# DhayaaAnbajagane/Baryonification

Hardware: AMD Instinct MI355X
Metric: halos/sec for BaryonifyShell NSIDE=1024 (1000000-halo synthetic catalog) (higher is better)
Workload: dtype f64 throughout in the parity-grade mode: f64 ring-row geometry, f64 pair math with 1e-11 elementary functions (fp32 seeds + one Newton step), f64 LDS accumulation, pix_offsets stored as two f32 arrays (hi + lo), f64 regrid geometry, f64 map

## Files before the change

baryonification_amd/csrc/bfgx_api.hip:

```cpp
#include <hip/hip_runtime.h>
#include <cmath>
#include <cstdarg>
#include <cstdio>
#include <algorithm>
#include <atomic>
#include <climits>
#include <cstdint>
#include <cstdlib>
#include <chrono>
#include <cstring>
#include <functional>
#include <map>
#include <memory>
#include <mutex>
#include <string>
#include <tuple>
#include <type_traits>
#include <vector>

#include "../../include/bfgx.h"

#include "bfgx_devmem.hpp"
#include "bfgx_tile_arena.hpp"
#include "bfgx_cosmo.hpp"
// ... 770 lines not shown
    {
        int cus = 0;
        if (hipDeviceGetAttribute(&cus, hipDeviceAttributeMultiprocessorCount, device) == hipSuccess && cus > 0) p->num_cus = cus;
    }
    p->nside = nside;
    p->max_halos = max_halos;
    p->hpx = make_hpx(nside);
    p->stream = (hipStream_t)hip_stream;
    auto bail = [&](int rc) { bfgx_plan_destroy(p); return rc; };

    const bfgx_table &t = model->table;
    if (int rc = upload_model(p->mem, p->stream, model, true, p->model, p->NC)) return bail(rc);
    plan_pick_precision(p, model);
    const size_t nh = (size_t)(max_halos > 0 ? max_halos : 1);
    if (p->mem.alloc(p->recs, nh)) return bail(alloc_fail("halo records"));
    if (p->NC > 4 && p->mem.alloc(p->rowsx, nh)) return bail(alloc_fail("corner rows"));
    if (int rc = plan_init_fast(p, t, nh)) return bail(rc);
    if (int rc = plan_init_binning(p, t, nh)) return bail(rc);
    if (int rc = plan_init_regrid(p)) return bail(rc);
    const ScanScratchLayout SL = scan_scratch_layout();
    int32_t *scan = nullptr;
    if (p->mem.alloc(scan, SL.total_words)) return bail(alloc_fail("tile scan scratch"));
    p->scan.bind(scan, SL);
    if (p->mem.alloc(p->tile_sums, 2 * (size_t)(p->tiling.ntiles + 1) + kFarEvalWgs)) return bail(alloc_fail("tile sums"));
    p->far_src.sums = p->tile_sums + 2 * (size_t)(p->tiling.ntiles + 1);
    if (hipMemsetAsync(p->far_src.sums, 0, sizeof(double) * kFarEvalWgs, p->stream) != hipSuccess) return bail(fail(BFGX_ERR_HIP, "hipMemset failed"));
    if (hipMemsetAsync(p->overflow, 0, sizeof(int32_t), p->stream) != hipSuccess) return bail(fail(BFGX_ERR_HIP, "hipMemset failed"));
    if (hipStreamSynchronize(p->stream) != hipSuccess) return bail(fail(BFGX_ERR_HIP, "stream sync failed"));
    *out = p;
    return BFGX_OK;
}

int bfgx_plan_timing_enable(bfgx_plan *p, int on)
{
    return p ? p->events.enable(on) : fail(BFGX_ERR_INVALID, "NULL plan");
}

int bfgx_plan_timing_read(bfgx_plan *p, double *ms_sum, int64_t *launches)
{
    return p ? p->events.read(p->device, p->stream, ms_sum, launches) : fail(BFGX_ERR_INVALID, "NULL argument");
}

void bfgx_plan_destroy(bfgx_plan *p)
{
    if (!p) return;
    (void)hipSetDevice(p->device);
    (void)hipStreamSynchronize(p->stream);
    p->events.destroy();
    p->mem.release();
// ... 171 lines not shown

}

constexpr int kSumTilesOneWg = 16384;
static int launch_tile_sums(bfgx_plan *p, int t0, int nt, double *sums_dev)
{
    const double *ts = p->tile_sums + 2 * (size_t)t0;
    const double *fs = p->far_src.sums;
    if (nt <= kSumTilesOneWg) hipLaunchKernelGGL(sum_tiles_kernel, dim3(1), dim3(256), 0, p->stream, nt, ts, sums_dev, fs, kFarEvalWgs);
    else {
        HIP_TRY(hipMemsetAsync(sums_dev, 0, 2 * sizeof(double), p->stream));
        hipLaunchKernelGGL(sum_tiles_multi_kernel, dim3(64), dim3(256), 0, p->stream, nt, ts, sums_dev, fs, kFarEvalWgs);
    }
    return BFGX_OK;
}

template <typename ACC, typename real, bool SPLIT = false>
static void launch_regrid_gather(bfgx_plan *p, const double *map_in_dev, const ACC *o, const ACC *o_lo, double *map_out_dev, double *ts, bool from_k1, double *sums_dev)
{
    const size_t lds = regrid3_lds_bytes(p->tiling.BR, p->tiling.W, sizeof(real)),
                 lds_walk = regrid3_lds_bytes(p->tiling.BR, p->tiling.W, sizeof(real), true, SPLIT ? sizeof(ACC) : sizeof(real));
    FarList far = p->far;
    far.overflow = p->arena.far_overflow_full;
    const int nt = p->tiling.ntiles, nfix = std::min(nt, 2 * p->num_cus), nwalk = std::min(nt, 4 * p->num_cus);
    const ReachArgs reach = reach_args(p, regrid_cap(p->hpx.nside));
    if (!from_k1)
        hipLaunchKernelGGL(tile_reach_kernel<ACC>, dim3(nt), dim3(256), 0, p->stream, p->hpx, p->tiling, o, p->arena.omax);
    hipLaunchKernelGGL(tile_apron_kernel, dim3((nt + 255) / 256), dim3(256), 0, p->stream, p->hpx, p->tiling, (const float *)p->arena.omax, 0,
                       reach.cap, 0, nt, p->tile_apron, p->arena.todo, p->regrid_lean);
    hipLaunchKernelGGL((tile_regrid3_kernel<ACC, real, 0, SPLIT>), dim3(std::min(nt, 8 * p->num_cus)), dim3(256), lds, p->stream, p->hpx, p->tiling, map_in_dev, o, o_lo,
                       map_out_dev, far, p->far_src, reach, ts, -1, nt, p->regrid_lean, (double *)nullptr);
    hipLaunchKernelGGL((tile_regrid3_kernel<ACC, real, 2, SPLIT>), dim3(nwalk), dim3(256), lds_walk, p->stream, p->hpx, p->tiling, map_in_dev, o, o_lo,
                       map_out_dev, far, p->far_src, reach, ts, -1, nt, p->arena.todo, (double *)nullptr);
    hipLaunchKernelGGL((regrid_far_eval_kernel<ACC, SPLIT>), dim3(kFarEvalWgs), dim3(256), 0, p->stream, p->hpx, p->tiling.rings, map_in_dev, o, o_lo, p->far_src, far);
    const bool many = nt > kSumTilesOneWg && sums_dev != nullptr && ts != nullptr;
    hipLaunchKernelGGL((tile_regrid3_kernel<ACC, real, 1, SPLIT>), dim3(nfix), dim3(256), lds, p->stream, p->hpx, p->tiling, map_in_dev, o, o_lo,
                       map_out_dev, far, p->far_src, reach, ts, -1, nt, p->arena.todo, many ? (double *)nullptr : sums_dev, p->regrid_lean);
    if (many) (void)launch_tile_sums(p, 0, nt, sums_dev);
}

extern "C" {

static int regrid_impl(bfgx_plan *p, const double *map_in_dev, const void *offsets_dev, const DispMode &m, double *map_out_dev, double *sums_dev,
                       bool from_k1)
{
    HIP_TRY(hipSetDevice(p->device));
    {
    KernelTimer kt(p, BFGX_K_REGRID);
    if (p->algo == 1) {
        if (!from_k1) HIP_TRY(hipMemsetAsync(p->arena.ctrl, 0, sizeof(RegridCtrl), p->stream));
        double *ts = sums_dev ? p->tile_sums : nullptr;
        if (m.split())
            launch_regrid_gather<float, double, true>(p, map_in_dev, (const float *)offsets_dev, m.lo(offsets_dev, p->hpx.npix),
                                                      map_out_dev, ts, from_k1, sums_dev);
        else if (m.fp64()) launch_regrid_gather<double, double>(p, map_in_dev, (const double *)offsets_dev, (const double *)nullptr, map_out_dev, ts, from_k1, sums_dev);
        else launch_regrid_gather<float, float>(p, map_in_dev, (const float *)offsets_dev, (const float *)nullptr, map_out_dev, ts, from_k1, sums_dev);
    } else {
        const unsigned grid = (unsigned)((p->hpx.npix + 255) / 256);
        if (m.fp64())
            hipLaunchKernelGGL(regrid_kernel<double>, dim3(grid), dim3(256), 0, p->stream, p->hpx, map_in_dev,
// ... 529 lines not shown
```

baryonification_amd/csrc/bfgx_regrid2.hpp:

```cpp
#pragma once
#include "bfgx_kernels.hpp"
#include "bfgx_scatter2.hpp"

namespace bfgx {

template <typename real>
struct alignas(16) RegRowC {
    real z, sth, dphi, inv_dphi;
    real c0, s0;
    real inv_dth_up, inv_dth_dn;
};
template <>
struct alignas(16) RegRowC<double> { double inv_dth_up, inv_dth_dn; };
template <typename real> struct RowGeom { real z, sth, dphi, inv_dphi, c0, s0, inv_dth_up, inv_dth_dn; };
__device__ inline RowGeom<float> row_geom(const RegRow *, const RegRowC<float> *rowc, int t)
{
    const RegRowC<float> c = rowc[t];
    return RowGeom<float>{c.z, c.sth, c.dphi, c.inv_dphi, c.c0, c.s0, c.inv_dth_up, c.inv_dth_dn};
}
__device__ inline RowGeom<double> row_geom(const RegRow *rows, const RegRowC<double> *rowc, int t)
{
    const RegRow &r = rows[t];
    const RegRowC<double> c = rowc[t];
    return RowGeom<double>{r.z, r.sth, r.dphi, r.inv_dphi, r.c0, r.s0, c.inv_dth_up, c.inv_dth_dn};
// ... 11 lines not shown
    __device__ inline double theta(int ir) const { return rows[ir - rth0].theta; }
    __device__ inline GenRing ring(int ir) const
    {
        const int t2 = ir - rth0;
        if (t2 >= 0 && t2 < LR + 2) { const RegRow &r2 = rows[t2]; return GenRing{r2.theta, r2.inv_dphi, r2.nr, r2.shf != 0}; }
        const RingRec &g2 = rings[ir];
        return GenRing{g2.theta, g2.inv_dphi, g2.nr, g2.shifted != 0};
    }
    __device__ inline GenSrc source(int ti, int x) const
    {
        const RegRow &rw = rows[ti];
        return GenSrc{rw.theta, rw.z, rw.sth, rw.dphi, rth0 + ti, rw.ks + x, rw.shf != 0};
    }
};
constexpr int kGenWalk = 17;
struct GenTable {
    const RingRec *__restrict__ rings; int lo_, hi_;
    __device__ inline int lo() const { return lo_; }
    __device__ inline int hi() const { return hi_; }
    __device__ inline double theta(int ir) const { return rings[ir].theta; }
    __device__ inline GenRing ring(int ir) const { const RingRec &g2 = rings[ir]; return GenRing{g2.theta, g2.inv_dphi, g2.nr, g2.shifted != 0}; }
};

template <typename RS>
__device__ inline void regrid_targets_generic(const Hpx &h, const RS &rs, const GenSrc &src, double o0, double o1, double o2, int tr[4], int tk[4], double w[4])
{
    const int nl4 = (int)(4 * h.nside);
    const double z = src.z, sth = src.sth;
    const double phi = ((double)src.k + (src.shf ? 0.5 : 0.0)) * src.dphi;
    double s, c;
    sincos_bounded(phi, s, c);
    const double nx = sth * c + o0, ny = sth * s + o1, nz = z + o2;
    const double xr = nx * c + ny * s, yr = ny * c - nx * s;
    const double inv = fast_rsq(nx * nx + ny * ny + nz * nz);
    const double zc = nz * inv;
    const double tq = yr * fast_rcp(xr);
    const double sn = fast_sqrt(xr * xr + yr * yr) * inv;
    const double q = sn * z - zc * sth;
    double theta, ph;
    if (xr > 0.0 && fabs(tq) <= 0.1 && fabs(q) <= 0.05) {
        ph = phi + atan_small(tq);
        theta = src.theta + asin_small(q);
    } else {
        theta = atan2_generic(sn, zc);
        ph = atan2_generic(ny, nx);
    }
    if (ph < 0) ph += kTwoPi;
    if (ph >= kTwoPi) ph -= kTwoPi;
    const int rlo = rs.lo(), rhi = rs.hi();
    const int rz = (int)ring_above(h, zc);
    int r1 = rz < rlo ? rlo : (rz > rhi ? rhi : rz);
    while (r1 > rlo && theta < rs.theta(r1)) --r1;
    while (r1 < rhi && theta >= rs.theta(r1 + 1)) ++r1;
    const bool in_window = (theta >= rs.theta(r1)) && (r1 < rhi) && (theta < rs.theta(r1 + 1));
    const int ir1 = in_window ? r1 : rz;
    const int ir2 = ir1 + 1;
    double theta1 = 0.0, theta2 = 0.0;
    for (int q4 = 0; q4 < 4; ++q4) { tr[q4] = 0; tk[q4] = 0; w[q4] = 0.0; }
#pragma unroll
    for (int half = 0; half < 2; ++half) {
        const int ir = half ? ir2 : ir1;
        if (half ? (ir < nl4) : (ir > 0)) {
            const GenRing g2 = rs.ring(ir);
            const int n2 = g2.nr;
            const double shd = g2.shf ? 0.5 : 0.0, invd = g2.inv_dphi, th = g2.theta;
            const double tmp = ph * invd - shd;
            int j1 = (int)floor(tmp);
            const double w1 = tmp - (double)j1;
            int j2 = j1 + 1;
            if (j1 < 0) j1 += n2;
            if (j2 >= n2) j2 -= n2;
            tr[2 * half] = ir; tr[2 * half + 1] = ir;
            tk[2 * half] = j1; tk[2 * half + 1] = j2;
            w[2 * half] = 1.0 - w1; w[2 * half + 1] = w1;
            if (half) theta2 = th; else theta1 = th;
        }
    }
    if (ir1 == 0) {
        const double wtheta = theta / theta2;
        w[2] *= wtheta; w[3] *= wtheta;
        const double fac = (1.0 - wtheta) * 0.25;
        w[0] = fac; w[1] = fac; w[2] += fac; w[3] += fac;
        tr[0] = 1; tr[1] = 1; tk[0] = (tk[2] + 2) & 3; tk[1] = (tk[3] + 2) & 3;
    } else if (ir2 == nl4) {
        const double wtheta = (theta - theta1) / (kPi - theta1);
        w[0] *= (1.0 - wtheta); w[1] *= (1.0 - wtheta);
        const double fac = wtheta * 0.25;
        w[0] += fac; w[1] += fac; w[2] = fac; w[3] = fac;
        tr[2] = nl4 - 1; tr[3] = nl4 - 1; tk[2] = (tk[0] + 2) & 3; tk[3] = (tk[1] + 2) & 3;
    } else {
        const double wtheta = (theta - theta1) * fast_rcp(theta2 - theta1);
        w[0] *= (1.0 - wtheta); w[1] *= (1.0 - wtheta);
        w[2] *= wtheta; w[3] *= wtheta;
    }
}

__device__ inline float abs_(float v) { return __builtin_fabsf(v); }
__device__ inline double abs_(double v) { return __builtin_fabs(v); }
template <typename real> struct RMath;
template <> struct RMath<float> {
    static __device__ inline float rcp(float x) { const float y = __builtin_amdgcn_rcpf(x); return y * __builtin_fmaf(-x, y, 2.0f); }
    static __device__ inline float inv_norm(float e) { return fma_(e, fma_(e, fma_(e, fma_(e, 0.2734375f, -0.3125f), 0.375f), -0.5f), 1.0f); }
    static __device__ inline float sqrt1pm1(float t2) { return t2 * fma_(t2, fma_(t2, 0.0625f, -0.125f), 0.5f); }
    static __device__ inline float asin_(float q) { const float q2 = q * q; return q * fma_(q2, fma_(q2, fma_(q2, (float)(15.0 / 336.0), 0.075f), (float)(1.0 / 6.0)), 1.0f); }
    static __device__ inline float atan_(float t) { const float t2 = t * t; return t * fma_(t2, fma_(t2, fma_(t2, fma_(t2, (float)(1.0 / 9.0), (float)(-1.0 / 7.0)), 0.2f), (float)(-1.0 / 3.0)), 1.0f); }
};
template <> struct RMath<double> {
    static __device__ inline double rcp(double x) { return fast_rcp(x); }
    static __device__ inline double inv_norm(double e) { return fast_rsq(1.0 + e); }
    static __device__ inline double sqrt1pm1(double t2) { const double h = 1.0 + t2; return t2 * fast_rcp(1.0 + h * fast_rsq(h)); }
    static __device__ inline double asin_(double q) { return asin_small(q); }
    static __device__ inline double atan_(double t) { return atan_small(t); }
};

struct RMathE {
    static __device__ inline double rcp(double x) { const double y = (double)__builtin_amdgcn_rcpf((float)x); return __builtin_fma(y, __builtin_fma(-x, y, 1.0), y); }
    static __device__ inline double inv_norm(double e)
    {
        const double x = 1.0 + e, y = (double)__builtin_amdgcn_rsqf((float)x);
// ... 24 lines not shown
    return R > kReachMax ? kReachMax : R;
}
__host__ __device__ inline double regrid_cap_for_rings(int64_t nside, int R)
{
    const double c = 0.999 * (double)R / (1.5 * (double)nside), cap = regrid_cap(nside);
    return (R >= kReachMax || c > cap) ? cap : c;
}

struct alignas(16) RowScan {
    int32_t start, nr, ks, span;
    float need2, cf2, lim2;
    int32_t klr;
};

struct FarList {
    unsigned long long *count;
    int64_t *pix;
    double *val;
    int64_t cap;
    int32_t *overflow;
};

constexpr int kFarEvalWgs = 1024;
struct FarSrc {
    unsigned int *count;
    int2 *ent;
    int64_t cap;
    double *sums;
};

__device__ inline bool far_src_append(const FarSrc &fs, int ring, int k)
{
    const unsigned long long act = __ballot(1);
    const int rank = (int)__builtin_amdgcn_mbcnt_hi((unsigned)(act >> 32), __builtin_amdgcn_mbcnt_lo((unsigned)act, 0u));
    const int leader = __ffsll((long long)act) - 1;
    unsigned base = 0;
    if (rank == 0) base = atomicAdd(fs.count, (unsigned)__popcll(act));
    base = (unsigned)__shfl((int)base, leader, kWave);
    const unsigned i = base + (unsigned)rank;
    if ((int64_t)i >= fs.cap) return false;
    fs.ent[i] = make_int2(ring, k);
    return true;
}

struct ReachArgs {
    const int32_t *apron;
// ... 206 lines not shown
    const int tx = nr_ ? ti : t1, ty = nr_ ? (down ? ti + 1 : ti - 1) : t1 + 1;
    int jx, jy; real wx, wy;
    if (nr_) {
        const real wall = dph * rc.inv_dphi, f = __builtin_floor(wall);
        wx = wall - f; jx = kown + (int)f;
    } else {
        other_ring(tx, jx, wx);
    }
    other_ring(ty, jy, wy);
    const int nrx = rows[tx].nr, nry = rows[ty].nr;
    int jx2 = jx + 1, jy2 = jy + 1;
    jx = jx < 0 ? jx + nrx : (jx >= nrx ? jx - nrx : jx);
    jx2 = jx2 < 0 ? jx2 + nrx : (jx2 >= nrx ? jx2 - nrx : jx2);
    jy = jy < 0 ? jy + nry : (jy >= nry ? jy - nry : jy);
    jy2 = jy2 < 0 ? jy2 + nry : (jy2 >= nry ? jy2 - nry : jy2);
    const real wtx = x_upper ? (real)1 - wtheta : wtheta, wty = (real)1 - wtx;
    tt[0] = tx; tt[1] = tx; tk[0] = jx; tk[1] = jx2;
    w[0] = ((real)1 - wx) * wtx; w[1] = wx * wtx;
    tt[2] = ty; tt[3] = ty; tk[2] = jy; tk[3] = jy2;
    w[2] = ((real)1 - wy) * wty; w[3] = wy * wty;
    return true;
}

template <typename RS>
__device__ inline double regrid_far_pixel(const Hpx &h, const RingRec *__restrict__ rings, const RS &rs, const GenSrc &src, double o0, double o1, double o2,
                                          double val, FarList far)
{
    int tr[4], tk[4];
    double w[4], tot = 0.0;
    regrid_targets_generic(h, rs, src, o0, o1, o2, tr, tk, w);
    const unsigned long long act = __ballot(1);
    const int rank = (int)__builtin_amdgcn_mbcnt_hi((unsigned)(act >> 32), __builtin_amdgcn_mbcnt_lo((unsigned)act, 0u));
    const int leader = __ffsll((long long)act) - 1;
    unsigned long long base = 0;
    if (rank == 0) base = atomicAdd(far.count, 4ull * (unsigned long long)__popcll(act));
    base = ((unsigned long long)(unsigned)__shfl((int)(base >> 32), leader, kWave) << 32) | (unsigned)__shfl((int)base, leader, kWave);
    for (int q4 = 0; q4 < 4; ++q4) {
        const double v = w[q4] * val;
        const unsigned long long i = base + 4ull * (unsigned long long)rank + (unsigned long long)q4;
        if ((int64_t)i < far.cap) { far.pix[i] = rings[tr[q4]].start + tk[q4]; far.val[i] = v; } else atomicOr(far.overflow, 1);
        tot += v;
    }
    return tot;
}

constexpr int kK2Occ = 4;
template <typename ACC, typename real, int PASS, bool SPLIT = false>
__global__ void __launch_bounds__(256, kK2Occ)
tile_regrid3_kernel(Hpx h, Tiling T, const double *__restrict__ map_in, const ACC *__restrict__ offsets, const ACC *__restrict__ offsets_lo,
                    double *__restrict__ map_out, FarList far, FarSrc fsrc, ReachArgs reach, double *__restrict__ tile_sums, int tile_off, int ntiles,
                    int *__restrict__ todo, double *__restrict__ sums_out, int *__restrict__ lean_reset = nullptr)
{
    static_assert(!SPLIT || (sizeof(ACC) == 4 && sizeof(real) == 8), "split pix_offsets: fp32 halves, fp64 geometry");
    extern __shared__ __align__(16) unsigned char smem[];
    const int NTmax = T.BR + 2 * kReachMax + 2;
    double *acc = reinterpret_cast<double *>(smem);
    RegRow *rows = reinterpret_cast<RegRow *>(acc + T.BR * T.W);
    RegRowC<real> *rowc = reinterpret_cast<RegRowC<real> *>(rows + NTmax);
    const int tid = threadIdx.x;
    const int nl4 = (int)(4 * h.nside);
    if (PASS == 1 && lean_reset != nullptr && blockIdx.x == 0 && tid == 0) *lean_reset = 0;
    if (PASS == 1 && sums_out != nullptr && blockIdx.x == 0) {
        double sa = 0.0, sb = 0.0;
        for (int i = tid; i < ntiles; i += 256) { sa += tile_sums[2 * (int64_t)i]; sb += tile_sums[2 * (int64_t)i + 1]; }
        for (int i = tid; i < kFarEvalWgs; i += 256) sb += fsrc.sums[i];
#pragma unroll
        for (int sft = kWave >> 1; sft > 0; sft >>= 1) { sa += __shfl_down(sa, sft, kWave); sb += __shfl_down(sb, sft, kWave); }
        double *red = reinterpret_cast<double *>(smem);
        if ((tid & (kWave - 1)) == 0) { red[2 * (tid / kWave)] = sa; red[2 * (tid / kWave) + 1] = sb; }
        __syncthreads();
        if (tid == 0) {
            double ta = 0.0, tb = 0.0;
            for (int w = 0; w < 256 / kWave; ++w) { ta += red[2 * w]; tb += red[2 * w + 1]; }
            sums_out[0] = ta; sums_out[1] = tb;
        }
        __syncthreads();
    }
    if (PASS == 1 && *far.overflow == 0) {
        const unsigned long long n = *far.count;
        for (unsigned long long i = (unsigned long long)blockIdx.x * 256 + tid; i < n; i += (unsigned long long)gridDim.x * 256)
            atomicAdd(map_out + far.pix[i], far.val[i]);
        return;
    }
    const bool listed = (PASS == 2 || PASS == 0) && todo != nullptr;
    if (listed) ntiles = min(todo[0], ntiles);
    for (int blk = blockIdx.x; blk < ntiles; blk += ((PASS == 0 && !listed) ? ntiles : (int)gridDim.x)) {
    const int tile = listed ? todo[1 + blk] : ((tile_off < 0) ? T.tile_order[blk] : tile_off + blk);
    const int band = T.tile_band[tile];
    const int nphi = T.band_nphi[band];
    const int tj = tile - T.band_tile0[band];
    const int i0 = 1 + band * T.BR;
    const int i1 = min(i0 + T.BR, nl4);
    double sum_in = 0.0, sum_out = 0.0;
    __syncthreads();

    const int R = (PASS == 2) ? reach.apron[2 * tile] : 1;
    const int kap = (PASS == 1 || nphi == 1) ? 0 : reach.apron[2 * tile + 1];
    if (PASS == 0 && reach.apron[2 * tile] > 1) continue;
    if (PASS == 0 && reach.apron[2 * tile] == 0) {
        const int lane = tid & (kWave - 1), wid = tid / kWave;
        for (int rr = wid; rr < i1 - i0; rr += 256 / kWave) {
            const int64_t st = T.rings[i0 + rr].start;
            const int nr = T.rings[i0 + rr].nr, ks = tile_ks(tj, nr, nphi), ke = tile_ks(tj + 1, nr, nphi);
            for (int k = ks + lane; k < ke; k += kWave) {
                const double v = map_in[st + k];
                const double dep = (v > 0.0) ? v : 0.0;
// ... 290 lines not shown
        const int n = rt.ke - rt.ks;
        for (int xx = lane; xx < n; xx += kWave) {
            const double v = acc[rr * T.W + xx];
            dst[xx] = v;
            sum_out += v;
        }
    }
    if (tile_sums) {
        __syncthreads();
#pragma unroll
        for (int sft = kWave >> 1; sft > 0; sft >>= 1) { sum_in += __shfl_down(sum_in, sft, kWave); sum_out += __shfl_down(sum_out, sft, kWave); }
        if (lane == 0) { acc[2 * wid] = sum_in; acc[2 * wid + 1] = sum_out; }
        __syncthreads();
        if (tid == 0) {
            double sa_ = 0.0, sb_ = 0.0;
            for (int wv = 0; wv < 256 / kWave; ++wv) { sa_ += acc[2 * wv]; sb_ += acc[2 * wv + 1]; }
            tile_sums[2 * (int64_t)tile] = sa_; tile_sums[2 * (int64_t)tile + 1] = sb_;
        }
    }
    __syncthreads();
    }
}

template <typename ACC, bool SPLIT>
__global__ void __launch_bounds__(256)
regrid_far_eval_kernel(Hpx h, const RingRec *__restrict__ rings, const double *__restrict__ map_in, const ACC *__restrict__ offsets,
                       const ACC *__restrict__ offsets_lo, FarSrc fsrc, FarList far)
{
    __shared__ double red[256 / kWave];
    const int tid = threadIdx.x;
    const unsigned listed = *fsrc.count;
    if (listed == 0u) {
        if (tid == 0) fsrc.sums[blockIdx.x] = 0.0;
        return;
    }
    const unsigned n = (int64_t)listed < fsrc.cap ? listed : (unsigned)fsrc.cap;
    if (listed > n && blockIdx.x == 0 && tid == 0) atomicAdd(far.count, 4ull * (unsigned long long)(listed - n));
    const int nl4 = (int)(4 * h.nside);
    double tot = 0.0;
    for (unsigned i = blockIdx.x * 256u + (unsigned)tid; i < n; i += (unsigned)kFarEvalWgs * 256u) {
        const int2 e = fsrc.ent[i];
        const RingRec &g = rings[e.x];
        const int64_t p = g.start + e.y;
        double o0 = (double)offsets[3 * p + 0], o1 = (double)offsets[3 * p + 1], o2 = (double)offsets[3 * p + 2];
        if (SPLIT) { o0 += (double)offsets_lo[3 * p + 0]; o1 += (double)offsets_lo[3 * p + 1]; o2 += (double)offsets_lo[3 * p + 2]; }
        const GenTable rs{rings, max(e.x - kGenWalk, 0), min(e.x + kGenWalk, nl4)};
        const GenSrc src{g.theta, g.z, g.sth, g.dphi, e.x, e.y, g.shifted != 0};
        tot += regrid_far_pixel(h, rings, rs, src, o0, o1, o2, map_in[p], far);
    }
#pragma unroll
    for (int sft = kWave >> 1; sft > 0; sft >>= 1) tot += __shfl_down(tot, sft, kWave);
    if ((tid & (kWave - 1)) == 0) red[tid / kWave] = tot;
    __syncthreads();
    if (tid == 0) {
        double t = 0.0;
        for (int w = 0; w < 256 / kWave; ++w) t += red[w];
        fsrc.sums[blockIdx.x] = t;
    }
}

__global__ void __launch_bounds__(256)
regrid_far_local_kernel(FarList far, double *__restrict__ out_slice, int64_t p0, int64_t p1, unsigned long long *__restrict__ foreign,
                        int ntiles = 0, const double *__restrict__ tile_sums = nullptr, double *__restrict__ sums = nullptr,
                        const double *__restrict__ far_sums = nullptr)
{
    if (tile_sums != nullptr && blockIdx.x == gridDim.x - 1) {
        __shared__ double sa[256 / kWave], sb[256 / kWave];
        double xa = 0.0, xb = 0.0;
        for (int t = threadIdx.x; t < ntiles; t += 256) { xa += tile_sums[2 * t]; xb += tile_sums[2 * t + 1]; }
        if (far_sums != nullptr) for (int t = threadIdx.x; t < kFarEvalWgs; t += 256) xb += far_sums[t];
#pragma unroll
        for (int sft = kWave >> 1; sft > 0; sft >>= 1) { xa += __shfl_down(xa, sft, kWave); xb += __shfl_down(xb, sft, kWave); }
        const int lane = threadIdx.x & (kWave - 1), wid = threadIdx.x / kWave;
        if (lane == 0) { sa[wid] = xa; sb[wid] = xb; }
        __syncthreads();
        if (threadIdx.x == 0) {
            double ta = 0.0, tb = 0.0;
            for (int w = 0; w < 256 / kWave; ++w) { ta += sa[w]; tb += sb[w]; }
            sums[0] = ta; sums[1] = tb;
        }
// ... 12 lines not shown
```

baryonification_amd/csrc/bfgx_shell_bands.inc:

```

extern "C" {

int bfgx_plan_bands(bfgx_plan *p, int32_t *nbands, int64_t *band_first_pixel)
{
    if (!p || !nbands) return fail(BFGX_ERR_INVALID, "NULL argument");
    *nbands = p->tiling.nbands;
    if (band_first_pixel)
        for (int b = 0; b <= p->tiling.nbands; ++b) band_first_pixel[b] = band_range(p, b, b).p0;
    return BFGX_OK;
}

int bfgx_plan_band_apron(bfgx_plan *p, int32_t band0, int32_t band1, int64_t *olo, int64_t *ohi)
{
    if (!p || !olo || !ohi) return fail(BFGX_ERR_INVALID, "NULL argument");
    if (int rc = check_band_range(p, band0, band1)) return rc;
    const int64_t i0 = 1 + (int64_t)p->tiling.BR * band0, i1 = 1 + (int64_t)p->tiling.BR * band1;
    *olo = ring_first_pixel(p->hpx, i0 - p->band_reach);
    *ohi = ring_first_pixel(p->hpx, i1 + p->band_reach);
    return BFGX_OK;
}

int bfgx_plan_reach_rings(bfgx_plan *p, double max_offset, int32_t *rings)
{
    if (!p || !rings) return fail(BFGX_ERR_INVALID, "NULL argument");
// ... 26 lines not shown
    if (!map_in_dev || !offsets_dev || !out_slice_dev) return fail(BFGX_ERR_INVALID, "NULL argument");
    if (olo > need_lo || ohi < need_hi || olo < 0 || ohi > p->hpx.npix)
        return fail(BFGX_ERR_INVALID, "pix_offsets range [%lld, %lld) does not cover the bands and %d ring(s) either side [%lld, %lld)",
                    (long long)olo, (long long)ohi, p->band_reach, (long long)need_lo, (long long)need_hi);
    HIP_TRY(hipSetDevice(p->device));
    if (reset_far) HIP_TRY(hipMemsetAsync(p->far.count, 0, kFarCountersBytes, p->stream));
    else if (!src_zeroed) HIP_TRY(hipMemsetAsync(p->far_src.count, 0, sizeof(uint32_t), p->stream));
    const BandRange r = band_range(p, band0, band1);
    {
        KernelTimer kt(p, BFGX_K_REGRID);
        const size_t lds = regrid3_lds_bytes(p->tiling.BR, p->tiling.W, m.fp64() ? sizeof(double) : sizeof(float), p->band_reach > 1,
                                             m.split() ? sizeof(float) : 0);
        double *out_base = out_slice_dev - r.p0;
        const ReachArgs reach = reach_args(p, regrid_cap_for_rings(p->hpx.nside, p->band_reach));
        hipLaunchKernelGGL(tile_apron_kernel, dim3((r.nt + 255) / 256), dim3(256), 0, p->stream, p->hpx, p->tiling, (const float *)nullptr,
                           p->band_reach, reach.cap, r.t0, r.nt, p->tile_apron, (int32_t *)nullptr);
        double *ts = sums_dev ? p->tile_sums : nullptr;
        const dim3 grid(r.nt), blk(256);
        int *none = nullptr;
#define BFGX_REGRID3(ACC, REAL, SPLIT, OL)                                                                                                     \
        do {                                                                                                                                    \
            const ACC *o = (const ACC *)offsets_dev - 3 * olo;                                                                                  \
            if (p->band_reach == 1) hipLaunchKernelGGL((tile_regrid3_kernel<ACC, REAL, 0, SPLIT>), grid, blk, lds, p->stream, p->hpx, p->tiling, map_in_dev, o, OL, \
                                                       out_base, p->far, p->far_src, reach, ts, r.t0, r.nt, none, (double *)nullptr);           \
            else hipLaunchKernelGGL((tile_regrid3_kernel<ACC, REAL, 2, SPLIT>), grid, blk, lds, p->stream, p->hpx, p->tiling, map_in_dev, o, OL, \
                                    out_base, p->far, p->far_src, reach, ts, r.t0, r.nt, none, (double *)nullptr);                              \
            hipLaunchKernelGGL((regrid_far_eval_kernel<ACC, SPLIT>), dim3(kFarEvalWgs), blk, 0, p->stream, p->hpx, p->tiling.rings, map_in_dev, o, OL, p->far_src, p->far); \
        } while (0)
        if (m.split()) BFGX_REGRID3(float, double, true, m.lo(offsets_dev, ohi - olo) - 3 * olo);
        else if (m.fp64()) BFGX_REGRID3(double, double, false, (const double *)nullptr);
        else BFGX_REGRID3(float, float, false, (const float *)nullptr);
#undef BFGX_REGRID3
        HIP_TRY(hipGetLastError());
    }
    if (sums_dev && !sums_later) {
        KernelTimer kt(p, BFGX_K_SUM);
        if (int rc = launch_tile_sums(p, r.t0, r.nt, sums_dev)) return rc;
        HIP_TRY(hipGetLastError());
    }
    return BFGX_OK;
}

static int offsets_bands(bfgx_plan *p, const bfgx_catalog *cat, int32_t band0, int32_t band1, void *slice, const DispMode &m)
{
    const BandRange r = band_range(p, band0, band1);
    TileLaunch k1;
    k1.tile_lo = r.t0; k1.tile_n = r.nt;
    if (int rc = launch_k0(p, cat, 1, m.fp64())) return rc;
    k1.omax = p->arena.omax;
    return launch_offsets(p, m, slice, r.p0, r.p1, k1);
// ... 120 lines not shown
```

baryonification_amd/csrc/bfgx_tile_arena.hpp:

```cpp
#pragma once
#include <cstddef>
#include <cstdint>

namespace bfgx {

struct RegridCtrl {
    unsigned long long far_count;
    uint32_t far_src_count;
    int32_t spare[3];
    int32_t far_overflow_full;
    int32_t todo_count;
};
static_assert(sizeof(RegridCtrl) == 32 && alignof(RegridCtrl) == 8, "RegridCtrl is eight words, the first two a 64-bit counter");
static_assert(offsetof(RegridCtrl, far_src_count) == 8 && offsetof(RegridCtrl, todo_count) == 28, "the two list counters are adjacent; the todo count is the last word");

constexpr size_t kFarCountersBytes = offsetof(RegridCtrl, far_src_count) + sizeof(uint32_t);
constexpr size_t kCtrlWords =sizeof(RegridCtrl) / sizeof(int32_t);
constexpr size_t round_up4(size_t words) { return (words + 3) & ~(size_t)3; }

struct TileArenaLayout {
    size_t cnt_a_pad, cnt_b, cur_b, tile_counter, omax, ctrl, far_overflow_full, todo, todo_list, band_overflow;
    size_t cursor_words;
    size_t zeroed_words;
    size_t tail_words;
    size_t total_words;
};

constexpr TileArenaLayout tile_arena_layout(size_t ntiles, size_t cnt_pad)
{
    const size_t blk = ntiles + 1;
    TileArenaLayout L{};
    L.cnt_a_pad = 0;
// ... 46 lines not shown
{
    ScanScratchLayout L{};
    L.block_tot = 0;
    L.block_off = L.block_tot + kScanBlocksRoom;
    L.total_words = L.block_off + kScanBlocksRoom;
    return L;
}
struct ScanScratch {
    int32_t *block_tot = nullptr, *block_off = nullptr;
    void bind(int32_t *b, const ScanScratchLayout &L) { block_tot = b + L.block_tot; block_off = b + L.block_off; }
};

template <size_t NT, size_t PAD>
struct TileArenaCheck {
    static constexpr TileArenaLayout L = tile_arena_layout(NT, PAD);
    static constexpr size_t blk = NT + 1;
    static constexpr bool unrounded = (NT * PAD) % 4 == 0;
    static constexpr size_t n3p = round_up4(3 * blk + 1);
    static_assert(L.cnt_a_pad == 0 && L.cnt_b >= NT * PAD, "the padded counters start the arena and hold ntiles * cnt_pad words");
    static_assert(L.cur_b == L.cnt_b + blk && L.cursor_words == blk && L.tile_counter == L.cur_b + L.cursor_words,
                  "cnt_b and cur_b: ntiles + 1 words each, and nothing else lies in the cursors' span");
    static_assert(L.omax == L.tile_counter + 1, "the |offset|^2 block follows the tile counter");
    static_assert(L.ctrl >= L.omax + blk && L.ctrl - (L.omax + blk) < 4, "the control words follow the three blocks and the tile counter, rounded up to four words");
    static_assert(L.far_overflow_full == L.ctrl + 6 && L.todo == L.ctrl + 7 && L.todo_list == L.todo + 1, "count (64 bits), source count, three spare, overflow, todo count, todo tiles");
    static_assert(L.band_overflow == L.todo_list + NT && L.total_words > L.band_overflow, "the banded overflow flag follows the todo tiles, inside the allocation");
    static_assert(L.zeroed_words == L.ctrl + kCtrlWords, "the zeroed span starts at the base and ends exactly after RegridCtrl");
    static_assert(L.zeroed_words % 4 == 0, "the zeroed span is a multiple of 16 bytes");
    static_assert(L.todo_list >= L.zeroed_words && L.band_overflow >= L.zeroed_words, "the step's memset touches neither the todo tiles nor the banded overflow flag");
    static_assert(L.ctrl % 2 == 0, "RegridCtrl's 64-bit counter is 8-byte aligned (the base is a device allocation)");
    static_assert(L.tail_words == L.total_words - L.ctrl && L.tail_words == NT + 12, "plan creation zeroes the control words and all behind them");
    static_assert(L.cnt_b == round_up4(NT * PAD) && (!unrounded || L.cnt_b == NT * PAD), "only a padded region that is no multiple of four words is rounded up");
    static_assert(L.tile_counter == L.cnt_b + 2 * blk && L.omax == L.cnt_b + 2 * blk + 1 && L.ctrl == L.cnt_b + n3p, "the three blocks, the tile counter between the second and the third");
    static_assert(L.zeroed_words == L.cnt_b + n3p + 8 && L.total_words == L.cnt_b + n3p + NT + 12, "lengths of the memset and of the allocation");
    static constexpr bool ok = true;
};
static_assert(TileArenaCheck<1, 32>::ok && TileArenaCheck<2, 32>::ok && TileArenaCheck<14, 32>::ok && TileArenaCheck<52, 32>::ok &&
              TileArenaCheck<6208, 32>::ok && TileArenaCheck<98560, 8>::ok && TileArenaCheck<393728, 2>::ok &&
              TileArenaCheck<3, 1>::ok && TileArenaCheck<12289, 1>::ok, "tile arena layout");

static_assert(scan_scratch_layout().block_tot == 0 && scan_scratch_layout().block_off == 1024 && scan_scratch_layout().total_words == 2048,
              "scan scratch: 1024 totals, then 1024 offsets: one word each per scan block");

}
```

Before: 952.6 million.

## Fuse far-list apply and tile-sum reduction into the far evaluator kernel

The far-pixel evaluator now atomically adds its contributions straight into the output map instead of writing a far list that the fix-up pass later replays. The final tile-sum reduction moves into the same kernel, finished by the last workgroup through a ticket counter. The evaluator also prefetches the next record in software, sizes its grid from npix, and the fix-up pass gets half as many workgroups. This removes a list write and reread plus a reduction step in the fix-up kernel, at the cost of more global atomics on the output map and a last-block reduction path.

```diff
diff --git a/baryonification_amd/csrc/bfgx_api.hip b/baryonification_amd/csrc/bfgx_api.hip
--- a/baryonification_amd/csrc/bfgx_api.hip
+++ b/baryonification_amd/csrc/bfgx_api.hip
@@ -816,9 +816,9 @@
     int32_t *scan = nullptr;
     if (p->mem.alloc(scan, SL.total_words)) return bail(alloc_fail("tile scan scratch"));
     p->scan.bind(scan, SL);
-    if (p->mem.alloc(p->tile_sums, 2 * (size_t)(p->tiling.ntiles + 1) + kFarEvalWgs)) return bail(alloc_fail("tile sums"));
+    if (p->mem.alloc(p->tile_sums, 2 * (size_t)(p->tiling.ntiles + 1) + 3 * (size_t)kFarEvalWgs)) return bail(alloc_fail("tile sums"));
     p->far_src.sums = p->tile_sums + 2 * (size_t)(p->tiling.ntiles + 1);
-    if (hipMemsetAsync(p->far_src.sums, 0, sizeof(double) * kFarEvalWgs, p->stream) != hipSuccess) return bail(fail(BFGX_ERR_HIP, "hipMemset failed"));
+    if (hipMemsetAsync(p->far_src.sums, 0, sizeof(double) * 3 * kFarEvalWgs, p->stream) != hipSuccess) return bail(fail(BFGX_ERR_HIP, "hipMemset failed"));
     if (hipMemsetAsync(p->overflow, 0, sizeof(int32_t), p->stream) != hipSuccess) return bail(fail(BFGX_ERR_HIP, "hipMemset failed"));
     if (hipStreamSynchronize(p->stream) != hipSuccess) return bail(fail(BFGX_ERR_HIP, "stream sync failed"));
     *out = p;
@@ -1036,20 +1036,22 @@
                  lds_walk = regrid3_lds_bytes(p->tiling.BR, p->tiling.W, sizeof(real), true, SPLIT ? sizeof(ACC) : sizeof(real));
     FarList far = p->far;
     far.overflow = p->arena.far_overflow_full;
-    const int nt = p->tiling.ntiles, nfix = std::min(nt, 2 * p->num_cus), nwalk = std::min(nt, 4 * p->num_cus);
+    const int nt = p->tiling.ntiles, nfix = std::min(nt, p->num_cus), nwalk = std::min(nt, 4 * p->num_cus);
     const ReachArgs reach = reach_args(p, regrid_cap(p->hpx.nside));
     if (!from_k1)
         hipLaunchKernelGGL(tile_reach_kernel<ACC>, dim3(nt), dim3(256), 0, p->stream, p->hpx, p->tiling, o, p->arena.omax);
     hipLaunchKernelGGL(tile_apron_kernel, dim3((nt + 255) / 256), dim3(256), 0, p->stream, p->hpx, p->tiling, (const float *)p->arena.omax, 0,
                        reach.cap, 0, nt, p->tile_apron, p->arena.todo, p->regrid_lean);
     hipLaunchKernelGGL((tile_regrid3_kernel<ACC, real, 0, SPLIT>), dim3(std::min(nt, 8 * p->num_cus)), dim3(256), lds, p->stream, p->hpx, p->tiling, map_in_dev, o, o_lo,
-                       map_out_dev, far, p->far_src, reach, ts, -1, nt, p->regrid_lean, (double *)nullptr);
+                       map_out_dev, far, p->far_src, reach, ts, -1, nt, p->regrid_lean);
     hipLaunchKernelGGL((tile_regrid3_kernel<ACC, real, 2, SPLIT>), dim3(nwalk), dim3(256), lds_walk, p->stream, p->hpx, p->tiling, map_in_dev, o, o_lo,
-                       map_out_dev, far, p->far_src, reach, ts, -1, nt, p->arena.todo, (double *)nullptr);
-    hipLaunchKernelGGL((regrid_far_eval_kernel<ACC, SPLIT>), dim3(kFarEvalWgs), dim3(256), 0, p->stream, p->hpx, p->tiling.rings, map_in_dev, o, o_lo, p->far_src, far);
+                       map_out_dev, far, p->far_src, reach, ts, -1, nt, p->arena.todo);
     const bool many = nt > kSumTilesOneWg && sums_dev != nullptr && ts != nullptr;
+    const FarFinish fin{map_out_dev, ts, nt, (many || ts == nullptr) ? (double *)nullptr : sums_dev, p->far_src.sums + kFarEvalWgs, &p->arena.ctrl->far_ticket, p->regrid_lean};
+    hipLaunchKernelGGL((regrid_far_eval_kernel<ACC, SPLIT, true>), dim3(far_eval_wgs(p->hpx.npix)), dim3(256), 0, p->stream, p->hpx, p->tiling.rings, map_in_dev, o, o_lo, p->far_src,
+                       far, fin);
     hipLaunchKernelGGL((tile_regrid3_kernel<ACC, real, 1, SPLIT>), dim3(nfix), dim3(256), lds, p->stream, p->hpx, p->tiling, map_in_dev, o, o_lo,
-                       map_out_dev, far, p->far_src, reach, ts, -1, nt, p->arena.todo, many ? (double *)nullptr : sums_dev, p->regrid_lean);
+                       map_out_dev, far, p->far_src, reach, ts, -1, nt, p->arena.todo);
     if (many) (void)launch_tile_sums(p, 0, nt, sums_dev);
 }
 
diff --git a/baryonification_amd/csrc/bfgx_regrid2.hpp b/baryonification_amd/csrc/bfgx_regrid2.hpp
--- a/baryonification_amd/csrc/bfgx_regrid2.hpp
+++ b/baryonification_amd/csrc/bfgx_regrid2.hpp
@@ -57,10 +57,24 @@
     __device__ inline GenRing ring(int ir) const { const RingRec &g2 = rings[ir]; return GenRing{g2.theta, g2.inv_dphi, g2.nr, g2.shifted != 0}; }
 };
 
-template <typename RS>
-__device__ inline void regrid_targets_generic(const Hpx &h, const RS &rs, const GenSrc &src, double o0, double o1, double o2, int tr[4], int tk[4], double w[4])
-{
-    const int nl4 = (int)(4 * h.nside);
+struct GenGuess {
+    const RingRec *__restrict__ rings; int lo_, hi_, g;
+    double th0, th1, id0, id1; int nr0, nr1; bool sh0, sh1;
+    __device__ inline int lo() const { return lo_; }
+    __device__ inline int hi() const { return hi_; }
+    __device__ inline double theta(int ir) const { return ir == g ? th0 : (ir == g + 1 ? th1 : rings[ir].theta); }
+    __device__ inline GenRing ring(int ir) const
+    {
+        if (ir == g) return GenRing{th0, id0, nr0, sh0};
+        if (ir == g + 1) return GenRing{th1, id1, nr1, sh1};
+        const RingRec &g2 = rings[ir];
+        return GenRing{g2.theta, g2.inv_dphi, g2.nr, g2.shifted != 0};
+    }
+};
+
+struct GenPos { double theta, ph; int rz; };
+__device__ inline GenPos regrid_generic_position(const Hpx &h, const GenSrc &src, double o0, double o1, double o2)
+{
     const double z = src.z, sth = src.sth;
     const double phi = ((double)src.k + (src.shf ? 0.5 : 0.0)) * src.dphi;
     double s, c;
@@ -82,9 +96,18 @@
     }
     if (ph < 0) ph += kTwoPi;
     if (ph >= kTwoPi) ph -= kTwoPi;
+    return GenPos{theta, ph, (int)ring_above(h, zc)};
+}
+__device__ inline int regrid_generic_guess(int rz, int rlo, int rhi) { return rz < rlo ? rlo : (rz > rhi ? rhi : rz); }
+
+template <typename RS>
+__device__ inline void regrid_generic_targets(const Hpx &h, const RS &rs, const GenPos &pos, int tr[4], int tk[4], double w[4])
+{
+    const int nl4 = (int)(4 * h.nside);
+    const double theta = pos.theta, ph = pos.ph;
     const int rlo = rs.lo(), rhi = rs.hi();
-    const int rz = (int)ring_above(h, zc);
-    int r1 = rz < rlo ? rlo : (rz > rhi ? rhi : rz);
+    const int rz = pos.rz;
+    int r1 = regrid_generic_guess(rz, rlo, rhi);
     while (r1 > rlo && theta < rs.theta(r1)) --r1;
     while (r1 < rhi && theta >= rs.theta(r1 + 1)) ++r1;
     const bool in_window = (theta >= rs.theta(r1)) && (r1 < rhi) && (theta < rs.theta(r1 + 1));
@@ -130,6 +153,12 @@
     }
 }
 
+template <typename RS>
+__device__ inline void regrid_targets_generic(const Hpx &h, const RS &rs, const GenSrc &src, double o0, double o1, double o2, int tr[4], int tk[4], double w[4])
+{
+    regrid_generic_targets(h, rs, regrid_generic_position(h, src, o0, o1, o2), tr, tk, w);
+}
+
 __device__ inline float abs_(float v) { return __builtin_fabsf(v); }
 __device__ inline double abs_(double v) { return __builtin_fabs(v); }
 template <typename real> struct RMath;
@@ -200,6 +229,7 @@
 };
 
 constexpr int kFarEvalWgs = 1024;
+__host__ __device__ inline int far_eval_wgs(int64_t npix) { const int64_t w = npix / 1024; return w < 1 ? 1 : (w > kFarEvalWgs ? kFarEvalWgs : (int)w); }
 struct FarSrc {
     unsigned int *count;
     int2 *ent;
@@ -452,23 +482,31 @@
     return true;
 }
 
-template <typename RS>
-__device__ inline double regrid_far_pixel(const Hpx &h, const RingRec *__restrict__ rings, const RS &rs, const GenSrc &src, double o0, double o1, double o2,
-                                          double val, FarList far)
-{
-    int tr[4], tk[4];
-    double w[4], tot = 0.0;
-    regrid_targets_generic(h, rs, src, o0, o1, o2, tr, tk, w);
-    const unsigned long long act = __ballot(1);
-    const int rank = (int)__builtin_amdgcn_mbcnt_hi((unsigned)(act >> 32), __builtin_amdgcn_mbcnt_lo((unsigned)act, 0u));
-    const int leader = __ffsll((long long)act) - 1;
+template <bool APPLY>
+__device__ inline double regrid_far_pixel(const Hpx &h, const int tr[4], const int tk[4], const double w[4], double val, FarList far,
+                                          double *__restrict__ map_out, bool apply)
+{
+    double tot = 0.0;
     unsigned long long base = 0;
-    if (rank == 0) base = atomicAdd(far.count, 4ull * (unsigned long long)__popcll(act));
-    base = ((unsigned long long)(unsigned)__shfl((int)(base >> 32), leader, kWave) << 32) | (unsigned)__shfl((int)base, leader, kWave);
+    int rank = 0;
+    if (!APPLY) {
+        const unsigned long long act = __ballot(1);
+        rank = (int)__builtin_amdgcn_mbcnt_hi((unsigned)(act >> 32), __builtin_amdgcn_mbcnt_lo((unsigned)act, 0u));
+        const int leader = __ffsll((long long)act) - 1;
+        if (rank == 0) base = atomicAdd(far.count, 4ull * (unsigned long long)__popcll(act));
+        base = ((unsigned long long)(unsigned)__shfl((int)(base >> 32), leader, kWave) << 32) | (unsigned)__shfl((int)base, leader, kWave);
+    }
     for (int q4 = 0; q4 < 4; ++q4) {
         const double v = w[q4] * val;
-        const unsigned long long i = base + 4ull * (unsigned long long)rank + (unsigned long long)q4;
-        if ((int64_t)i < far.cap) { far.pix[i] = rings[tr[q4]].start + tk[q4]; far.val[i] = v; } else atomicOr(far.overflow, 1);
+        int64_t st, nr; bool shf;
+        ring_info_small(h, tr[q4], st, nr, shf);
+        const int64_t pix = st + tk[q4];
+        if (APPLY) {
+            if (apply && (uint64_t)pix < (uint64_t)h.npix) atomicAdd(map_out + pix, v);
+        } else {
+            const unsigned long long i = base + 4ull * (unsigned long long)rank + (unsigned long long)q4;
+            if ((int64_t)i < far.cap) { far.pix[i] = pix; far.val[i] = v; } else atomicOr(far.overflow, 1);
+        }
         tot += v;
     }
     return tot;
@@ -479,7 +517,7 @@
 __global__ void __launch_bounds__(256, kK2Occ)
 tile_regrid3_kernel(Hpx h, Tiling T, const double *__restrict__ map_in, const ACC *__restrict__ offsets, const ACC *__restrict__ offsets_lo,
                     double *__restrict__ map_out, FarList far, FarSrc fsrc, ReachArgs reach, double *__restrict__ tile_sums, int tile_off, int ntiles,
-                    int *__restrict__ todo, double *__restrict__ sums_out, int *__restrict__ lean_reset = nullptr)
+                    int *__restrict__ todo)
 {
     static_assert(!SPLIT || (sizeof(ACC) == 4 && sizeof(real) == 8), "split pix_offsets: fp32 halves, fp64 geometry");
     extern __shared__ __align__(16) unsigned char smem[];
@@ -489,29 +527,7 @@
     RegRowC<real> *rowc = reinterpret_cast<RegRowC<real> *>(rows + NTmax);
     const int tid = threadIdx.x;
     const int nl4 = (int)(4 * h.nside);
-    if (PASS == 1 && lean_reset != nullptr && blockIdx.x == 0 && tid == 0) *lean_reset = 0;
-    if (PASS == 1 && sums_out != nullptr && blockIdx.x == 0) {
-        double sa = 0.0, sb = 0.0;
-        for (int i = tid; i < ntiles; i += 256) { sa += tile_sums[2 * (int64_t)i]; sb += tile_sums[2 * (int64_t)i + 1]; }
-        for (int i = tid; i < kFarEvalWgs; i += 256) sb += fsrc.sums[i];
-#pragma unroll
-        for (int sft = kWave >> 1; sft > 0; sft >>= 1) { sa += __shfl_down(sa, sft, kWave); sb += __shfl_down(sb, sft, kWave); }
-        double *red = reinterpret_cast<double *>(smem);
-        if ((tid & (kWave - 1)) == 0) { red[2 * (tid / kWave)] = sa; red[2 * (tid / kWave) + 1] = sb; }
-        __syncthreads();
-        if (tid == 0) {
-            double ta = 0.0, tb = 0.0;
-            for (int w = 0; w < 256 / kWave; ++w) { ta += red[2 * w]; tb += red[2 * w + 1]; }
-            sums_out[0] = ta; sums_out[1] = tb;
-        }
-        __syncthreads();
-    }
-    if (PASS == 1 && *far.overflow == 0) {
-        const unsigned long long n = *far.count;
-        for (unsigned long long i = (unsigned long long)blockIdx.x * 256 + tid; i < n; i += (unsigned long long)gridDim.x * 256)
-            atomicAdd(map_out + far.pix[i], far.val[i]);
-        return;
-    }
+    if (PASS == 1 && *far.overflow == 0) return;
     const bool listed = (PASS == 2 || PASS == 0) && todo != nullptr;
     if (listed) ntiles = min(todo[0], ntiles);
     for (int blk = blockIdx.x; blk < ntiles; blk += ((PASS == 0 && !listed) ? ntiles : (int)gridDim.x)) {
@@ -848,40 +864,121 @@
     }
 }
 
+template <typename ACC> struct FarRec { int ring, k, shifted; ACC h0, h1, h2, l0, l1, l2; double val, theta, z, sth, dphi; };
 template <typename ACC, bool SPLIT>
-__global__ void __launch_bounds__(256)
+__device__ inline FarRec<ACC> far_rec_load(const Hpx &h, const RingRec *__restrict__ rings, const double *__restrict__ map_in, const ACC *__restrict__ offsets,
+                                           const ACC *__restrict__ offsets_lo, int2 e)
+{
+    int64_t st, nr; bool shf;
+    ring_info_small(h, e.x, st, nr, shf);
+    const int64_t p = st + e.y;
+    const RingRec &g = rings[e.x];
+    FarRec<ACC> r;
+    r.ring = e.x; r.k = e.y; r.shifted = g.shifted;
+    r.h0 = offsets[3 * p + 0]; r.h1 = offsets[3 * p + 1]; r.h2 = offsets[3 * p + 2];
+    r.l0 = r.l1 = r.l2 = (ACC)0;
+    if (SPLIT) { r.l0 = offsets_lo[3 * p + 0]; r.l1 = offsets_lo[3 * p + 1]; r.l2 = offsets_lo[3 * p + 2]; }
+    r.val = map_in[p];
+    r.theta = g.theta; r.z = g.z; r.sth = g.sth; r.dphi = g.dphi;
+    return r;
+}
+struct FarFinish {
+    double *map_out;
+    const double *tile_sums;
+    int ntiles;
+    double *sums_out;
+    double *part;
+    unsigned int *ticket;
+    int *lean_reset;
+};
+template <typename ACC, bool SPLIT, bool APPLY = false>
+__global__ void __launch_bounds__(256, 4)
 regrid_far_eval_kernel(Hpx h, const RingRec *__restrict__ rings, const double *__restrict__ map_in, const ACC *__restrict__ offsets,
-                       const ACC *__restrict__ offsets_lo, FarSrc fsrc, FarList far)
-{
-    __shared__ double red[256 / kWave];
+                       const ACC *__restrict__ offsets_lo, FarSrc fsrc, FarList far, FarFinish fin = FarFinish{})
+{
+    __shared__ double red[3 * (256 / kWave) + 1];
     const int tid = threadIdx.x;
     const unsigned listed = *fsrc.count;
-    if (listed == 0u) {
-        if (tid == 0) fsrc.sums[blockIdx.x] = 0.0;
-        return;
-    }
-    const unsigned n = (int64_t)listed < fsrc.cap ? listed : (unsigned)fsrc.cap;
-    if (listed > n && blockIdx.x == 0 && tid == 0) atomicAdd(far.count, 4ull * (unsigned long long)(listed - n));
-    const int nl4 = (int)(4 * h.nside);
-    double tot = 0.0;
-    for (unsigned i = blockIdx.x * 256u + (unsigned)tid; i < n; i += (unsigned)kFarEvalWgs * 256u) {
-        const int2 e = fsrc.ent[i];
-        const RingRec &g = rings[e.x];
-        const int64_t p = g.start + e.y;
-        double o0 = (double)offsets[3 * p + 0], o1 = (double)offsets[3 * p + 1], o2 = (double)offsets[3 * p + 2];
-        if (SPLIT) { o0 += (double)offsets_lo[3 * p + 0]; o1 += (double)offsets_lo[3 * p + 1]; o2 += (double)offsets_lo[3 * p + 2]; }
-        const GenTable rs{rings, max(e.x - kGenWalk, 0), min(e.x + kGenWalk, nl4)};
-        const GenSrc src{g.theta, g.z, g.sth, g.dphi, e.x, e.y, g.shifted != 0};
-        tot += regrid_far_pixel(h, rings, rs, src, o0, o1, o2, map_in[p], far);
-    }
-#pragma unroll
-    for (int sft = kWave >> 1; sft > 0; sft >>= 1) tot += __shfl_down(tot, sft, kWave);
-    if ((tid & (kWave - 1)) == 0) red[tid / kWave] = tot;
-    __syncthreads();
-    if (tid == 0) {
-        double t = 0.0;
-        for (int w = 0; w < 256 / kWave; ++w) t += red[w];
-        fsrc.sums[blockIdx.x] = t;
+    double tile_a = 0.0, tile_b = 0.0, tot = 0.0;
+    if constexpr (APPLY) {
+        if (fin.sums_out != nullptr)
+            for (int t = (int)blockIdx.x + (int)gridDim.x * tid; t < fin.ntiles; t += (int)gridDim.x * 256) {
+                tile_a += fin.tile_sums[2 * (int64_t)t]; tile_b += fin.tile_sums[2 * (int64_t)t + 1];
+            }
+    }
+    if (listed != 0u) {
+        const unsigned n = (int64_t)listed < fsrc.cap ? listed : (unsigned)fsrc.cap;
+        const bool apply = APPLY && *far.overflow == 0;
+        const unsigned long long uncounted = 4ull * (unsigned long long)(APPLY ? listed : listed - n);
+        if (uncounted != 0ull && blockIdx.x == 0 && tid == 0) atomicAdd(far.count, uncounted);
+        const int nl4 = (int)(4 * h.nside);
+        const unsigned stride = gridDim.x * 256u;
+        unsigned i = blockIdx.x * 256u + (unsigned)tid;
+        int2 e1 = make_int2(0, 0);
+        FarRec<ACC> cur = {};
+        if (i < n) {
+            const int2 e0 = fsrc.ent[i];
+            if (n - i > stride) e1 = fsrc.ent[i + stride];
+            cur = far_rec_load<ACC, SPLIT>(h, rings, map_in, offsets, offsets_lo, e0);
+        }
+        for (; i < n; i += stride) {
+            FarRec<ACC> nxt = {};
+            int2 e2 = make_int2(0, 0);
+            if (n - i > stride) nxt = far_rec_load<ACC, SPLIT>(h, rings, map_in, offsets, offsets_lo, e1);
+            if (n - i > 2u * stride) e2 = fsrc.ent[i + 2u * stride];
+            double o0 = (double)cur.h0, o1 = (double)cur.h1, o2 = (double)cur.h2;
+            if (SPLIT) { o0 += (double)cur.l0; o1 += (double)cur.l1; o2 += (double)cur.l2; }
+            const GenSrc src{cur.theta, cur.z, cur.sth, cur.dphi, cur.ring, cur.k, cur.shifted != 0};
+            const GenPos pos = regrid_generic_position(h, src, o0, o1, o2);
+            const int rlo = max(cur.ring - kGenWalk, 0), rhi = min(cur.ring + kGenWalk, nl4);
+            const int g = regrid_generic_guess(pos.rz, rlo, rhi);
+            const RingRec &ga = rings[g], &gb = rings[min(g + 1, nl4)];
+            const GenGuess rs{rings, rlo, rhi, g, ga.theta, gb.theta, ga.inv_dphi, gb.inv_dphi, ga.nr, gb.nr, ga.shifted != 0, gb.shifted != 0};
+            int tr[4], tk[4];
+            double w[4];
+            regrid_generic_targets(h, rs, pos, tr, tk, w);
+            tot += regrid_far_pixel<APPLY>(h, tr, tk, w, cur.val, far, fin.map_out, apply);
+            cur = nxt; e1 = e2;
+        }
+    }
+    const bool finish = APPLY && fin.sums_out != nullptr;
+    double wg_tot = 0.0, wg_a = 0.0, wg_b = 0.0;
+    if (listed != 0u || finish) {
+#pragma unroll
+        for (int sft = kWave >> 1; sft > 0; sft >>= 1) {
+            tot += __shfl_down(tot, sft, kWave); tile_a += __shfl_down(tile_a, sft, kWave); tile_b += __shfl_down(tile_b, sft, kWave);
+        }
+        if ((tid & (kWave - 1)) == 0) { red[3 * (tid / kWave)] = tot; red[3 * (tid / kWave) + 1] = tile_a; red[3 * (tid / kWave) + 2] = tile_b; }
+        __syncthreads();
+        if (tid == 0) for (int w = 0; w < 256 / kWave; ++w) { wg_tot += red[3 * w]; wg_a += red[3 * w + 1]; wg_b += red[3 * w + 2]; }
+    }
+    if (tid == 0) __hip_atomic_store(fsrc.sums + blockIdx.x, wg_tot, __ATOMIC_RELAXED, __HIP_MEMORY_SCOPE_AGENT);
+    if constexpr (APPLY) {
+        if (fin.lean_reset != nullptr && blockIdx.x == 0 && tid == 0) *fin.lean_reset = 0;
+        if (!finish) return;
+        int *last = reinterpret_cast<int *>(red + 3 * (256 / kWave));
+        if (tid == 0) {
+            __hip_atomic_store(fin.part + blockIdx.x, wg_a, __ATOMIC_RELAXED, __HIP_MEMORY_SCOPE_AGENT);
+            __hip_atomic_store(fin.part + kFarEvalWgs + blockIdx.x, wg_b + wg_tot, __ATOMIC_RELAXED, __HIP_MEMORY_SCOPE_AGENT);
+            asm volatile("s_waitcnt vmcnt(0)" ::: "memory");
+            *last = __hip_atomic_fetch_add(fin.ticket, 1u, __ATOMIC_RELAXED, __HIP_MEMORY_SCOPE_AGENT) == gridDim.x - 1u;
+        }
+        __syncthreads();
+        if (*last == 0) return;
+        double sa = 0.0, sb = 0.0;
+        for (unsigned t = (unsigned)tid; t < gridDim.x; t += 256u) {
+            sa += __hip_atomic_load(fin.part + t, __ATOMIC_RELAXED, __HIP_MEMORY_SCOPE_AGENT);
+            sb += __hip_atomic_load(fin.part + kFarEvalWgs + t, __ATOMIC_RELAXED, __HIP_MEMORY_SCOPE_AGENT);
+        }
+#pragma unroll
+        for (int sft = kWave >> 1; sft > 0; sft >>= 1) { sa += __shfl_down(sa, sft, kWave); sb += __shfl_down(sb, sft, kWave); }
+        if ((tid & (kWave - 1)) == 0) { red[2 * (tid / kWave)] = sa; red[2 * (tid / kWave) + 1] = sb; }
+        __syncthreads();
+        if (tid == 0) {
+            double ta = 0.0, tb = 0.0;
+            for (int w = 0; w < 256 / kWave; ++w) { ta += red[2 * w]; tb += red[2 * w + 1]; }
+            fin.sums_out[0] = ta; fin.sums_out[1] = tb;
+        }
     }
 }
 
diff --git a/baryonification_amd/csrc/bfgx_shell_bands.inc b/baryonification_amd/csrc/bfgx_shell_bands.inc
--- a/baryonification_amd/csrc/bfgx_shell_bands.inc
+++ b/baryonification_amd/csrc/bfgx_shell_bands.inc
@@ -72,10 +72,10 @@
         do {                                                                                                                                    \
             const ACC *o = (const ACC *)offsets_dev - 3 * olo;                                                                                  \
             if (p->band_reach == 1) hipLaunchKernelGGL((tile_regrid3_kernel<ACC, REAL, 0, SPLIT>), grid, blk, lds, p->stream, p->hpx, p->tiling, map_in_dev, o, OL, \
-                                                       out_base, p->far, p->far_src, reach, ts, r.t0, r.nt, none, (double *)nullptr);           \
+                                                       out_base, p->far, p->far_src, reach, ts, r.t0, r.nt, none);                               \
             else hipLaunchKernelGGL((tile_regrid3_kernel<ACC, REAL, 2, SPLIT>), grid, blk, lds, p->stream, p->hpx, p->tiling, map_in_dev, o, OL, \
-                                    out_base, p->far, p->far_src, reach, ts, r.t0, r.nt, none, (double *)nullptr);                              \
-            hipLaunchKernelGGL((regrid_far_eval_kernel<ACC, SPLIT>), dim3(kFarEvalWgs), blk, 0, p->stream, p->hpx, p->tiling.rings, map_in_dev, o, OL, p->far_src, p->far); \
+                                    out_base, p->far, p->far_src, reach, ts, r.t0, r.nt, none);                                                  \
+            hipLaunchKernelGGL((regrid_far_eval_kernel<ACC, SPLIT>), dim3(far_eval_wgs(p->hpx.npix)), blk, 0, p->stream, p->hpx, p->tiling.rings, map_in_dev, o, OL, p->far_src, p->far); \
         } while (0)
         if (m.split()) BFGX_REGRID3(float, double, true, m.lo(offsets_dev, ohi - olo) - 3 * olo);
         else if (m.fp64()) BFGX_REGRID3(double, double, false, (const double *)nullptr);
diff --git a/baryonification_amd/csrc/bfgx_tile_arena.hpp b/baryonification_amd/csrc/bfgx_tile_arena.hpp
--- a/baryonification_amd/csrc/bfgx_tile_arena.hpp
+++ b/baryonification_amd/csrc/bfgx_tile_arena.hpp
@@ -7,7 +7,8 @@
 struct RegridCtrl {
     unsigned long long far_count;
     uint32_t far_src_count;
-    int32_t spare[3];
+    uint32_t far_ticket;
+    int32_t spare[2];
     int32_t far_overflow_full;
     int32_t todo_count;
 };
@@ -100,7 +101,7 @@
                   "cnt_b and cur_b: ntiles + 1 words each, and nothing else lies in the cursors' span");
     static_assert(L.omax == L.tile_counter + 1, "the |offset|^2 block follows the tile counter");
     static_assert(L.ctrl >= L.omax + blk && L.ctrl - (L.omax + blk) < 4, "the control words follow the three blocks and the tile counter, rounded up to four words");
-    static_assert(L.far_overflow_full == L.ctrl + 6 && L.todo == L.ctrl + 7 && L.todo_list == L.todo + 1, "count (64 bits), source count, three spare, overflow, todo count, todo tiles");
+    static_assert(L.far_overflow_full == L.ctrl + 6 && L.todo == L.ctrl + 7 && L.todo_list == L.todo + 1, "count (64 bits), source count, evaluator ticket, two spare, overflow, todo count, todo tiles");
     static_assert(L.band_overflow == L.todo_list + NT && L.total_words > L.band_overflow, "the banded overflow flag follows the todo tiles, inside the allocation");
     static_assert(L.zeroed_words == L.ctrl + kCtrlWords, "the zeroed span starts at the base and ends exactly after RegridCtrl");
     static_assert(L.zeroed_words % 4 == 0, "the zeroed span is a multiple of 16 bytes");
```

Result: no change. 958.8 million, median of 6 (+0.7%).
